# stella-cv/stella_vslam

Hardware: NVIDIA H100
Metric: frames/sec (ORB+match+local BA) @1920x1080, 2000 kpts (higher is better)
Workload: dtype u8

## Files before the change

### stella_vslam_b200/csrc/orb_kernels.cu

```cuda
#include <cuda.h>

#include <algorithm>
#include <cmath>
#include <new>
#include <vector>

#include "common.cuh"
#include "track_chain.cuh"
#include "util_trig.cuh"

namespace b200 {
namespace orb {

constexpr int kMaxLevels = 16;
constexpr int kBorder = 19;
constexpr int kCell = 64;
constexpr int kOverlap = 6;
constexpr int kTileMax = kCell + kOverlap;
constexpr int kTilePitch = 80;

struct LevelGeom {
    int w, h, pitch;
    unsigned long long offset;
    float sf;
    int nx, ny;
    double delta_x, delta_y;
    int grid_base;
    int ncols;
    float size;
    int tab_x, tab_y;
};

struct Geom {
    int num_levels;
    int grid_cells;
    int ini_thr, min_thr;
    LevelGeom lv[kMaxLevels];
};

struct CellDesc {
    unsigned short level, i, j, min_x, min_y, w, h, pad;
};

struct RawKp {
    short x, y;
    unsigned char m;
    unsigned char level;
    unsigned short pad;
};

struct ResizeTap {
    short ofs, w0, w1, pad;
};

struct Images {
    const unsigned char* img0;
    unsigned long long pitch0, fstride0;
    unsigned char* pyr;
    unsigned long long pyr_fstride;
};

__device__ __forceinline__ const unsigned char* level_ptr(const Images& im, const Geom& g, int level, int frame, int* pitch) {
    if (level == 0) {
        *pitch = (int)im.pitch0;
        return im.img0 + (size_t)frame * im.fstride0;
    }
    *pitch = g.lv[level].pitch;
    return im.pyr + (size_t)frame * im.pyr_fstride + g.lv[level].offset;
}

struct TmapSet {
    CUtensorMap m[kMaxLevels];
};

__device__ __forceinline__ unsigned smem_u32(const void* p) { return (unsigned)__cvta_generic_to_shared(p); }

__device__ __forceinline__ void mbar_init(unsigned long long* bar, unsigned count) {
    asm volatile("mbarrier.init.shared::cta.b64 [%0], %1;" ::"r"(smem_u32(bar)), "r"(count));
    asm volatile("fence.mbarrier_init.release.cluster;" ::: "memory");
}
__device__ __forceinline__ void mbar_expect_tx(unsigned long long* bar, unsigned bytes) {
    asm volatile("mbarrier.arrive.expect_tx.shared::cta.b64 _, [%0], %1;" ::"r"(smem_u32(bar)), "r"(bytes) : "memory");
}
__device__ __forceinline__ void mbar_wait(unsigned long long* bar, unsigned parity) {
    asm volatile(
        "{\n\t.reg .pred p;\n\t"
        "WAIT_%=:\n\t"
        "mbarrier.try_wait.parity.shared::cta.b64 p, [%0], %1;\n\t"
        "@p bra DONE_%=;\n\t"
        "bra WAIT_%=;\n\t"
        "DONE_%=:\n\t}" ::"r"(smem_u32(bar)),
        "r"(parity)
        : "memory");
}
__device__ __forceinline__ void tma_load_3d(void* smem_dst, const CUtensorMap* tmap, int x, int y, int z, unsigned long long* bar) {
    asm volatile("cp.async.bulk.tensor.3d.shared::cluster.global.mbarrier::complete_tx::bytes [%0], [%1, {%2, %3, %4}], [%5];" ::"r"(
                     smem_u32(smem_dst)),
                 "l"(reinterpret_cast<unsigned long long>(tmap)), "r"(x), "r"(y), "r"(z), "r"(smem_u32(bar))
                 : "memory");
}

constexpr int kRzRows = 8;

__global__ void __launch_bounds__(128) resize_kernel(const __grid_constant__ Geom g, Images im, const ResizeTap* __restrict__ taps, int level) {
    const LevelGeom& L = g.lv[level];
    const int frame = blockIdx.z;
    int spitch;
    const unsigned char* src = level_ptr(im, g, level - 1, frame, &spitch);
    unsigned char* dst = im.pyr + (size_t)frame * im.pyr_fstride + L.offset;
    const int sw = g.lv[level - 1].w, sh = g.lv[level - 1].h;
    const int dxq = (blockIdx.x * blockDim.x + threadIdx.x) * 4;
    const int dy0 = blockIdx.y * kRzRows;
    if (dxq >= L.pitch) return;
    const int n_valid = min(4, L.w - dxq);
    const unsigned store_mask = n_valid >= 4 ? 0xFFFFFFFFu : (n_valid <= 0 ? 0u : ((1u << (8 * n_valid)) - 1u));
    int ofs[4], ofs1[4];
    unsigned w01[4];
#pragma unroll
    for (int k = 0; k < 4; ++k) {
        const ResizeTap t = taps[L.tab_x + min(dxq + k, L.w - 1)];
        ofs[k] = t.ofs;
        ofs1[k] = min((int)t.ofs + 1, sw - 1);
        w01[k] = ((unsigned)t.w0 & 0xFFFFu) | ((unsigned)t.w1 << 16);
    }
    int rowA = -1, rowB = -1;
    unsigned hA[4] = {0, 0, 0, 0}, hB[4] = {0, 0, 0, 0};
    auto hrow = [&](int sy, unsigned (&h)[4]) {
        const unsigned char* r = src + (size_t)sy * spitch;
#pragma unroll
        for (int k = 0; k < 4; ++k) h[k] = __dp2a_lo(w01[k], (unsigned)r[ofs[k]] | ((unsigned)r[ofs1[k]] << 8), 0u) >> 4;
    };
    const int dy_end = min(dy0 + kRzRows, L.h);
    unsigned char* drow = dst + (size_t)dy0 * L.pitch + dxq;
    for (int dy = dy0; dy < dy_end; ++dy, drow += L.pitch) {
        const ResizeTap ty = taps[L.tab_y + dy];
        const int s0 = min(max((int)ty.ofs, 0), sh - 1), s1 = min(max((int)ty.ofs + 1, 0), sh - 1);
        if (s0 != rowA) {
            if (s0 == rowB) {
#pragma unroll
                for (int k = 0; k < 4; ++k) hA[k] = hB[k];
            } else {
                hrow(s0, hA);
            }
            rowA = s0;
        }
        if (s1 != rowB) {
            if (s1 == rowA) {
#pragma unroll
                for (int k = 0; k < 4; ++k) hB[k] = hA[k];
            } else {
                hrow(s1, hB);
            }
            rowB = s1;
        }
        const unsigned b0 = (unsigned)(int)ty.w0 << 16, b1 = (unsigned)(int)ty.w1 << 16;
        unsigned out = 0;
#pragma unroll
        for (int k = 0; k < 4; ++k) out |= ((__umulhi(b0, hA[k]) + __umulhi(b1, hB[k]) + 2u) >> 2) << (8 * k);
        *reinterpret_cast<unsigned*>(drow) = out & store_mask;
    }
}

__device__ __forceinline__ bool has_run9(unsigned m16) {
    unsigned m = m16 | (m16 << 16);
    unsigned x = m & (m >> 1);
    x &= x >> 2;
    x &= x >> 4;
    x &= m >> 8;
    return (x & 0xFFFFu) != 0;
}

#define FAST_OFF(k, P)                                                                                              \
    ((k) == 0 ? 3 * (P) : (k) == 1 ? 3 * (P) + 1 : (k) == 2 ? 2 * (P) + 2 : (k) == 3 ? (P) + 3 : (k) == 4 ? 3      \
     : (k) == 5 ? -(P) + 3 : (k) == 6 ? -2 * (P) + 2 : (k) == 7 ? -3 * (P) + 1 : (k) == 8 ? -3 * (P)              \
     : (k) == 9 ? -3 * (P)-1 : (k) == 10 ? -2 * (P)-2 : (k) == 11 ? -(P)-3 : (k) == 12 ? -3                        \
     : (k) == 13 ? (P)-3 : (k) == 14 ? 2 * (P)-2 : 3 * (P)-1)

__device__ __forceinline__ bool mask_zero(const unsigned char* mask, unsigned long long mask_pitch, unsigned y, unsigned x, float sf) {
    const int r = (int)__fmul_rn((float)y, sf), c = (int)__fmul_rn((float)x, sf);
    return mask[(size_t)r * mask_pitch + c] == 0;
}

__device__ __forceinline__ unsigned fast_m4(const unsigned (&w)[7][3], unsigned neg_tlow2) {
    constexpr int DX[16] = {0, 1, 2, 3, 3, 3, 2, 1, 0, -1, -2, -3, -3, -3, -2, -1};
    constexpr int DY[16] = {3, 3, 2, 1, 0, -1, -2, -3, -3, -3, -2, -1, 0, 1, 2, 3};
    unsigned pe[16], po[16];
    const unsigned ve = __byte_perm(w[3][1], 0, 0x4240), vo = __byte_perm(w[3][1], 0, 0x4341);
    auto extract = [&](int k) {
        const int dx = DX[k], r = DY[k] + 3;
        unsigned x;
        if (dx == 0) x = w[r][1];
        else if (dx > 0) x = __byte_perm(w[r][1], w[r][2], 0x3210 + 0x1111 * dx);
        else x = __byte_perm(w[r][0], w[r][1], 0x3210 + 0x1111 * (4 + dx));
        pe[k] = __byte_perm(x, 0, 0x4240);
        po[k] = __byte_perm(x, 0, 0x4341);
    };
#pragma unroll
    for (int k = 0; k < 16; ++k) extract(k);
    unsigned res[2];
#pragma unroll
    for (int half = 0; half < 2; ++half) {
        const unsigned* p = half ? po : pe;
        const unsigned v = half ? vo : ve;
        unsigned mx3[16], mn3[16];
#pragma unroll
        for (int k = 0; k < 16; ++k) {
            mx3[k] = __vimax3_u16x2(p[k], p[(k + 1) & 15], p[(k + 2) & 15]);
            mn3[k] = __vimin3_u16x2(p[k], p[(k + 1) & 15], p[(k + 2) & 15]);
        }
        unsigned mx9[16], mn9[16];
#pragma unroll
        for (int k = 0; k < 16; ++k) {
            mx9[k] = __vimax3_u16x2(mx3[k], mx3[(k + 3) & 15], mx3[(k + 6) & 15]);
            mn9[k] = __vimin3_u16x2(mn3[k], mn3[(k + 3) & 15], mn3[(k + 6) & 15]);
        }
        unsigned a = __vimin3_u16x2(mx9[0], mx9[1], mx9[2]), b = __vimax3_u16x2(mn9[0], mn9[1], mn9[2]);
#pragma unroll
        for (int k = 3; k < 15; k += 2) {
            a = __vimin3_u16x2(a, mx9[k], mx9[k + 1]);
            b = __vimax3_u16x2(b, mn9[k], mn9[k + 1]);
        }
        a = __vminu2(a, mx9[15]);
        b = __vmaxu2(b, mn9[15]);
        const unsigned dark = __vsub2(v, a), bright = __vsub2(b, v);
        const unsigned m = __vimax_s16x2_relu(dark, bright);
        res[half] = __viaddmax_s16x2_relu(m, neg_tlow2, 0u);
    }
    return __byte_perm(res[0], res[1], 0x6240);
}

__device__ __forceinline__ unsigned fast_candidates4(const unsigned (&w)[7][3], unsigned tlow2) {
    const unsigned x0 = w[6][1], x8 = w[0][1];
    const unsigned x4 = __byte_perm(w[3][1], w[3][2], 0x6543), x12 = __byte_perm(w[3][0], w[3][1], 0x4321);
    unsigned r[2];
#pragma unroll
    for (int half = 0; half < 2; ++half) {
        const unsigned sel = half ? 0x4341u : 0x4240u;
        const unsigned p0 = __byte_perm(x0, 0, sel), p8 = __byte_perm(x8, 0, sel), p4 = __byte_perm(x4, 0, sel), p12 = __byte_perm(x12, 0, sel);
        const unsigned v = __byte_perm(w[3][1], 0, sel);
        const unsigned hi = __vminu2(__vmaxu2(p0, p8), __vmaxu2(p4, p12));
        const unsigned lo = __vmaxu2(__vminu2(p0, p8), __vminu2(p4, p12));
        const unsigned vt = v + tlow2, lot = lo + tlow2;
        r[half] = (__vmaxu2(hi, vt) ^ vt) | (__vmaxu2(v, lot) ^ lot);
    }
    return ((r[0] & 0xFFFFu) ? 1u : 0u) | ((r[1] & 0xFFFFu) ? 2u : 0u) | ((r[0] >> 16) ? 4u : 0u) | ((r[1] >> 16) ? 8u : 0u);
}

__device__ __forceinline__ int fast_score1(const unsigned char* __restrict__ p, int t_low) {
    constexpr int OFF[16] = {3 * kTilePitch,     3 * kTilePitch + 1,  2 * kTilePitch + 2,  kTilePitch + 3,  3,  -kTilePitch + 3, -2 * kTilePitch + 2, -3 * kTilePitch + 1,
                             -3 * kTilePitch,    -3 * kTilePitch - 1, -2 * kTilePitch - 2, -kTilePitch - 3, -3, kTilePitch - 3,  2 * kTilePitch - 2,  3 * kTilePitch - 1};
    unsigned c[16];
#pragma unroll
    for (int k = 0; k < 16; ++k) c[k] = (unsigned)p[OFF[k]] * 0xFFFF0001u + 0x00FF0000u;
    const int v = p[0];
    unsigned mx3[16];
#pragma unroll
    for (int k = 0; k < 16; ++k) mx3[k] = __vimax3_s16x2(c[k], c[(k + 1) & 15], c[(k + 2) & 15]);
    unsigned ab = 0x00FF00FFu;
#pragma unroll
    for (int k = 0; k < 16; k += 2)
        ab = __vimin3_s16x2(ab, __vimax3_s16x2(mx3[k], mx3[(k + 3) & 15], mx3[(k + 6) & 15]),
                            __vimax3_s16x2(mx3[k + 1], mx3[(k + 4) & 15], mx3[(k + 7) & 15]));
    const int a = (int)(ab & 0xFFFFu), b = 255 - (int)(ab >> 16);
    const int at = a + t_low, vt = v + t_low;
    return (max(v, at) - at) + (max(b, vt) - vt);
}

constexpr int kFastThreads = 256;
constexpr int kTileRows = kTileMax + 2;
constexpr int kRawPitch = 96;

template <bool kUseTma>
__global__ void __launch_bounds__(kFastThreads) fast_cells_kernel(const __grid_constant__ Geom g, const __grid_constant__ TmapSet tmaps, Images im,
                                                                  const CellDesc* __restrict__ cells, const unsigned char* __restrict__ mask,
                                                                  unsigned long long mask_pitch, unsigned long long* __restrict__ grid,
                                                                  int arena_frame0, int* __restrict__ raw_corners) {
    __shared__ __align__(16) unsigned char tile[kTileRows * kTilePitch];
    __shared__ __align__(16) unsigned char mmap[kTileRows * kTilePitch];
    __shared__ __align__(128) unsigned char raw[kUseTma ? kTileRows * kRawPitch : 16];
    __shared__ __align__(8) unsigned long long tma_bar;
    __shared__ int skip;
    __shared__ unsigned short cand[(kTileMax - 6) * (kTileMax - 6)];
    __shared__ int n_cand;

    const CellDesc cd = cells[blockIdx.x];
    const int frame = blockIdx.y;
    const int level = cd.level;
    const LevelGeom& L = g.lv[level];
    const int cw = cd.w, ch = cd.h;
    const int tid = threadIdx.x;

    if (tid == 0) {
        int s = 0;
        if (mask) {
            const unsigned max_x = cd.min_x + cw, max_y = cd.min_y + ch;
            s = mask_zero(mask, mask_pitch, cd.min_y, cd.min_x, L.sf) || mask_zero(mask, mask_pitch, max_y, cd.min_x, L.sf)
                || mask_zero(mask, mask_pitch, cd.min_y, max_x, L.sf) || mask_zero(mask, mask_pitch, max_y, max_x, L.sf);
        }
        skip = s;
        n_cand = 0;
    }
    if constexpr (kUseTma) {
        if (tid == 0) {
            mbar_init(&tma_bar, 1);
            mbar_expect_tx(&tma_bar, kTileRows * kRawPitch);
            tma_load_3d(raw, &tmaps.m[level], (int)cd.min_x - 3, (int)cd.min_y, frame + (level ? arena_frame0 : 0), &tma_bar);
        }
        __syncthreads();
        mbar_wait(&tma_bar, 0);
        for (int idx = tid; idx < kTileRows * (kTilePitch / 4); idx += kFastThreads) {
            const int y = idx / (kTilePitch / 4), q = idx - y * (kTilePitch / 4);
            const unsigned* rw = reinterpret_cast<const unsigned*>(raw + y * kRawPitch) + q;
            reinterpret_cast<unsigned*>(tile)[idx] = __funnelshift_r(rw[0], rw[1], 16);
            reinterpret_cast<unsigned*>(mmap)[idx] = 0u;
        }
        __syncthreads();
    } else {
        int pitch;
        const unsigned char* src = level_ptr(im, g, level, frame, &pitch);
        src += (size_t)cd.min_y * pitch + cd.min_x;
        for (int idx = tid; idx < kTileRows * (kTilePitch / 4); idx += kFastThreads) {
            const int y = idx / (kTilePitch / 4), c4 = (idx - y * (kTilePitch / 4)) * 4;
            unsigned v = 0;
            if (y < ch) {
#pragma unroll
                for (int b = 0; b < 4; ++b) {
                    const int x = c4 + b - 1;
                    if (x >= 0 && x < cw) v |= (unsigned)src[(size_t)y * pitch + x] << (8 * b);
                }
            }
            reinterpret_cast<unsigned*>(tile)[idx] = v;
            reinterpret_cast<unsigned*>(mmap)[idx] = 0u;
        }
        __syncthreads();
    }
    if (skip) return;

    const int t_low = min(g.ini_thr, g.min_thr);
    const unsigned neg_tlow2 = (unsigned)((-t_low) & 0xFFFF) * 0x10001u;
    if (t_low <= 126) {
        const int wq = tid & 15, rg = tid >> 4;
        const int c0 = 4 + 4 * wq;
        const int lx0 = c0 - 1;
        const int y0 = 3 + 4 * rg;
        if (lx0 <= cw - 4 && y0 <= ch - 4) {
            const unsigned c7f = (unsigned)(0x7F - t_low) * 0x01010101u;
            auto gt = [&](unsigned d) { return (((d & 0x7F7F7F7Fu) + c7f) | d) & 0x80808080u; };
            unsigned ctr[10];
#pragma unroll
            for (int r = 0; r < 10; ++r) ctr[r] = *reinterpret_cast<const unsigned*>(tile + (y0 - 3 + r) * kTilePitch + c0);
            unsigned acc = 0;
#pragma unroll
            for (int i = 0; i < 4; ++i) {
                const unsigned* row = reinterpret_cast<const unsigned*>(tile + (y0 + i) * kTilePitch + c0 - 4);
                const unsigned v = ctr[i + 3];
                const unsigned p4 = __byte_perm(v, row[2], 0x6543), p12 = __byte_perm(row[0], v, 0x4321);
                const unsigned gbits = (gt(__vabsdiffu4(ctr[i + 6], v)) | gt(__vabsdiffu4(ctr[i], v))) & (gt(__vabsdiffu4(p4, v)) | gt(__vabsdiffu4(p12, v)));
                acc |= gbits >> (7 - i);
            }
            const int nvalid = min(4, cw - 3 - lx0), nrows = min(4, ch - 3 - y0);
            acc &= (0xFFFFFFFFu >> (32 - 8 * nvalid)) & (((1u << nrows) - 1u) * 0x01010101u);
            if (acc) {
                int pos = atomicAdd(&n_cand, __popc(acc));
                const unsigned enc0 = (unsigned)((y0 << 8) | c0);
#pragma unroll
                for (int b = 0; b < 4; ++b) {
                    const unsigned nib = (acc >> (8 * b)) & 0xFu;
#pragma unroll
                    for (int i = 0; i < 4; ++i)
                        if ((nib >> i) & 1u) cand[pos + __popc(nib & ((1u << i) - 1u))] = (unsigned short)(enc0 + (unsigned)((i << 8) | b));
                    pos += __popc(nib);
                }
            }
        }
    } else {
        const int wq = tid & 15, rg = tid >> 4;
        const int c0 = 4 + 4 * wq;
        const int lx0 = c0 - 1;
        const int y0 = 3 + 4 * rg;
        if (lx0 <= cw - 4 && y0 <= ch - 4) {
            unsigned w[10][3];
#pragma unroll
            for (int r = 0; r < 10; ++r) {
                const int y = y0 - 3 + r;
                const unsigned* row = reinterpret_cast<const unsigned*>(tile + y * kTilePitch + c0 - 4);
                w[r][0] = row[0];
                w[r][1] = row[1];
                w[r][2] = row[2];
            }
            const int nvalid = min(4, cw - 3 - lx0);
            const unsigned keep = (1u << nvalid) - 1u;
            unsigned bits = 0;
#pragma unroll
            for (int i = 0; i < 4; ++i) {
                if (y0 + i <= ch - 4) {
                    unsigned ww[7][3];
#pragma unroll
                    for (int r = 0; r < 7; ++r) {
                        ww[r][0] = w[i + r][0];
                        ww[r][1] = w[i + r][1];
                        ww[r][2] = w[i + r][2];
                    }
                    bits |= (fast_candidates4(ww, (unsigned)t_low * 0x10001u) & keep) << (4 * i);
                }
            }
            if (bits) {
                int pos = atomicAdd(&n_cand, __popc(bits));
                while (bits) {
                    const int k = __ffs(bits) - 1;
                    bits &= bits - 1;
                    cand[pos++] = (unsigned short)(((y0 + (k >> 2)) << 8) | (c0 + (k & 3)));
                }
            }
        }
    }
    __syncthreads();
    {
        const int n = n_cand;
        for (int i = tid; i < n; i += kFastThreads) {
            const int e = cand[i], y = e >> 8, c = e & 0xFF;
            mmap[y * kTilePitch + c] = (unsigned char)fast_score1(tile + y * kTilePitch + c, t_low);
        }
    }
    __syncthreads();
    const int ini_rel = g.ini_thr - t_low, min_rel = g.min_thr - t_low;
    const int n_c = n_cand;
// ... 264 lines not shown
            for (int idx = lane; idx < kFdHpW * 5; idx += 32) {
                const int rb = idx / kFdHpW, c = idx - rb * kFdHpW;
                unsigned p[7];
#pragma unroll
                for (int t = 0; t < 7; ++t) p[t] = (4 * rb + t < kFdHpRows) ? S.hp[(4 * rb + t) * kFdHpW + c] : 0u;
#pragma unroll
                for (int i = 0; i < 4; ++i) {
                    unsigned e = __dp2a_lo(p[i], E01, 0u);
                    e = __dp2a_hi(p[i + 1], E01, e);
                    e = __dp2a_lo(p[i + 2], E23, e);
                    e = __dp2a_hi(p[i + 3], E23, e);
                    unsigned o = __dp2a_lo(p[i], O01, 0u);
                    o = __dp2a_hi(p[i + 1], O01, o);
                    o = __dp2a_lo(p[i + 2], O23, o);
                    o = __dp2a_hi(p[i + 3], O23, o);
                    S.blur[(8 * rb + 2 * i) * kFdHpW + c] = (unsigned char)min((e + 32768u) >> 16, 255u);
                    S.blur[(8 * rb + 2 * i + 1) * kFdHpW + c] = (unsigned char)min((o + 32768u) >> 16, 255u);
                }
            }
        }
        int m10 = 0, m01 = 0;
        if (lane < 31) {
            const int u = lane - 15, au = abs(u);
            const unsigned char* c = tile + 21 * kFdTileW + ox + 21 + u;
            int col = 0;
#pragma unroll
            for (int v = -15; v <= 15; ++v) {
                if (au <= c_umax[v < 0 ? -v : v]) {
                    const int val = c[v * kFdTileW];
                    col += val;
                    m01 += v * val;
                }
            }
            m10 = u * col;
        }
#pragma unroll
        for (int s2 = 16; s2 > 0; s2 >>= 1) {
            m10 += __shfl_xor_sync(0xFFFFFFFFu, m10, s2);
            m01 += __shfl_xor_sync(0xFFFFFFFFu, m01, s2);
        }
        const float angle = fast_atan2_deg((float)m01, (float)m10);
        __syncwarp();
        const float arad = (float)((double)angle * 3.14159265358979323846 / 180.0);
        const float ca = util_cos(arad), sa = util_sin(arad);
        const unsigned char* bc = S.blur + kFdR * kFdHpW + kFdR;
        unsigned val = 0;
#pragma unroll
        for (int b = 0; b < 8; ++b) {
            const float x0 = (float)(int)(signed char)(pat[b] & 0xFF), y0 = (float)(int)(signed char)((pat[b] >> 8) & 0xFF);
            const float x1 = (float)(int)(signed char)((pat[b] >> 16) & 0xFF), y1 = (float)(int)(signed char)(pat[b] >> 24);
            int r0 = __float2int_rn(__fadd_rn(__fmul_rn(x0, sa), __fmul_rn(y0, ca)));
            int c0 = __float2int_rn(__fsub_rn(__fmul_rn(x0, ca), __fmul_rn(y0, sa)));
            int r1 = __float2int_rn(__fadd_rn(__fmul_rn(x1, sa), __fmul_rn(y1, ca)));
            int c1 = __float2int_rn(__fsub_rn(__fmul_rn(x1, ca), __fmul_rn(y1, sa)));
            r0 = max(-kFdR, min(kFdR, r0)); c0 = max(-kFdR, min(kFdR, c0));
            r1 = max(-kFdR, min(kFdR, r1)); c1 = max(-kFdR, min(kFdR, c1));
            val |= (unsigned)(bc[r0 * kFdHpW + c0] < bc[r1 * kFdHpW + c1]) << b;
        }
        const size_t o = (size_t)frame * out_stride + k;
        descs[o * 32 + lane] = (unsigned char)val;
        if (lane == 0) {
            b200_keypoint_t kp;
            float x = (float)kx, y = (float)ky;
            if (level > 0) {
                x = __fmul_rn(x, L.sf);
                y = __fmul_rn(y, L.sf);
            }
            kp.x = x;
            kp.y = y;
            kp.size = L.size;
            kp.angle = angle;
            kp.response = (float)(rk.m - 1);
            kp.octave = level;
            kps[o] = kp;
        }
        __syncwarp();
    }
}

static inline short sat_short_rint(float v) {
    long r = lrintf(v);
    return (short)std::min(32767L, std::max(-32768L, r));
}
static inline int floor_to_int(float v) {
    int i = (int)v;
    return i - (v < (float)i);
}

typedef CUresult (*EncodeTiledFn)(CUtensorMap*, CUtensorMapDataType, cuuint32_t, void*, const cuuint64_t*, const cuuint64_t*, const cuuint32_t*,
                                  const cuuint32_t*, CUtensorMapInterleave, CUtensorMapSwizzle, CUtensorMapL2promotion, CUtensorMapFloatOOBfill);

static EncodeTiledFn encode_tiled_fn() {
    static EncodeTiledFn fn = nullptr;
    static bool tried = false;
    if (!tried) {
        tried = true;
        void* p = nullptr;
        cudaDriverEntryPointQueryResult q;
        if (cudaGetDriverEntryPointByVersion("cuTensorMapEncodeTiled", &p, 12000, cudaEnableDefault, &q) == cudaSuccess
            && q == cudaDriverEntryPointSuccess)
            fn = (EncodeTiledFn)p;
    }
    return fn;
}

static bool make_level_tmap(CUtensorMap* out, const void* base, int w, int h, size_t pitch, size_t fstride, int frames, int box_w = kRawPitch,
                            int box_h = kTileRows) {
    EncodeTiledFn fn = encode_tiled_fn();
    if (!fn) return false;
    if ((reinterpret_cast<unsigned long long>(base) & 15ull) || (pitch & 15) || (frames > 1 && (fstride & 15)) || w < 1 || h < 1) return false;
    const cuuint64_t dims[3] = {(cuuint64_t)w, (cuuint64_t)h, (cuuint64_t)std::max(frames, 1)};
    const cuuint64_t strides[2] = {(cuuint64_t)pitch, (cuuint64_t)(frames > 1 ? fstride : pitch * (size_t)h + ((16 - (pitch * (size_t)h) % 16) % 16))};
    const cuuint32_t box[3] = {(cuuint32_t)box_w, (cuuint32_t)box_h, 1};
    const cuuint32_t estr[3] = {1, 1, 1};
    return fn(out, CU_TENSOR_MAP_DATA_TYPE_UINT8, 3, const_cast<void*>(base), dims, strides, box, estr, CU_TENSOR_MAP_INTERLEAVE_NONE,
              CU_TENSOR_MAP_SWIZZLE_NONE, CU_TENSOR_MAP_L2_PROMOTION_NONE, CU_TENSOR_MAP_FLOAT_OOB_FILL_NONE)
           == CUDA_SUCCESS;
}

struct Extractor {
    b200_orb_params_t prm{};
    std::vector<float> mask_rects;
    cudaStream_t own_stream = nullptr, stream = nullptr, copy_stream = nullptr;
    cudaEvent_t ev[8] = {};
    std::vector<cudaEvent_t> chunk_events;
    cudaEvent_t chunk_event(int i) {
        while ((int)chunk_events.size() <= i) {
            cudaEvent_t e = nullptr;
            if (cudaEventCreateWithFlags(&e, cudaEventDisableTiming) != cudaSuccess) return nullptr;
            chunk_events.push_back(e);
        }
        return chunk_events[i];
    }
    bool timing = false;
    float stage_ms[6] = {};
    int width = 0, height = 0, batch_cap = 0;
    Geom geom{};
    std::vector<float> sf;
    int n_cells = 0, raw_stride = 0;
    size_t pyr_fstride = 0, img0_pitch = 0, img0_fstride = 0;
    unsigned char *d_img0 = nullptr, *d_pyr = nullptr, *d_rect_mask = nullptr, *d_user_mask = nullptr;
    CellDesc* d_cells = nullptr;
    ResizeTap* d_taps = nullptr;
    unsigned long long* d_grid = nullptr;
    RawKp* d_raw = nullptr;
    int *d_counts = nullptr, *d_level_counts = nullptr, *d_raw_corners = nullptr;
    b200_keypoint_t* d_kps = nullptr;
    unsigned char* d_descs = nullptr;
    int* h_counts = nullptr;
    int last_batch = 0;
    const unsigned char* last_img0 = nullptr;
    size_t last_pitch0 = 0, last_fstride0 = 0;
    bool rect_mask_ready = false;
    TmapSet tmaps{};
    TmapSet tmaps_desc{};
    bool tmaps_ok = false, last_used_tma = false;
    int tmap_frames = 0;
    b200_keypoint_t* out_kps = nullptr;
    unsigned char* out_descs = nullptr;
    int* out_counts = nullptr;
    int out_stride = 0;
    b200_keypoint_t* res_kps() const { return out_kps ? out_kps : d_kps; }
    unsigned char* res_descs() const { return out_kps ? out_descs : d_descs; }
    int* res_counts() const { return out_kps ? out_counts : d_counts; }
    int res_stride() const { return out_kps ? out_stride : raw_stride; }

    void free_arenas() {
        cudaFree(d_img0); cudaFree(d_pyr); cudaFree(d_rect_mask); cudaFree(d_user_mask);
        cudaFree(d_cells); cudaFree(d_taps); cudaFree(d_grid); cudaFree(d_raw);
        cudaFree(d_counts); cudaFree(d_level_counts); cudaFree(d_raw_corners); cudaFree(d_kps); cudaFree(d_descs);
        if (h_counts) cudaFreeHost(h_counts);
        d_img0 = d_pyr = d_rect_mask = d_user_mask = nullptr;
        d_cells = nullptr; d_taps = nullptr; d_grid = nullptr; d_raw = nullptr;
        d_counts = d_level_counts = d_raw_corners = nullptr; d_kps = nullptr; d_descs = nullptr; h_counts = nullptr;
        rect_mask_ready = false;
    }

    static int level_geometry(const b200_orb_params_t& prm, int w, int h, Geom& g, std::vector<float>& sf) {
        const int nl = prm.num_levels;
        sf.assign(nl, 1.0f);
        for (int l = 1; l < nl; ++l) sf[l] = prm.scale_factor * sf[l - 1];
        g = Geom{};
        g.num_levels = nl;
        g.ini_thr = std::min(255, std::max(0, prm.ini_fast_thr));
        g.min_thr = std::min(255, std::max(0, prm.min_fast_thr));
        const unsigned min_area_sqrt = (unsigned)std::sqrt((double)prm.min_area);
        unsigned long long off = 0;
        int grid_base = 0;
        for (int l = 0; l < nl; ++l) {
            LevelGeom& L = g.lv[l];
            if (l == 0) {
                L.w = w;
                L.h = h;
            } else {
                const double scale = sf[l];
                L.w = (int)std::round(w * 1.0 / scale);
                L.h = (int)std::round(h * 1.0 / scale);
            }
            if (L.w < 1 || L.h < 1) {
                set_error("pyramid level %d of a %dx%d image is empty", l, w, h);
                return B200_ERR_INVALID;
            }
            L.pitch = round_up(L.w, 64);
            L.offset = off;
            off += round_up((unsigned long long)L.pitch * L.h, 256ull);
            L.sf = sf[l];
            L.size = (float)(unsigned)(31 * sf[l]);
            L.grid_base = grid_base;
            if (L.w > 2 * kBorder && L.h > 2 * kBorder) {
                const int span_x = L.w - 2 * kBorder, span_y = L.h - 2 * kBorder;
                const double s = (double)((float)min_area_sqrt / sf[l]);
                L.nx = (int)(unsigned)std::ceil(span_x / s);
                L.ny = (int)(unsigned)std::ceil(span_y / s);
                L.delta_x = (double)span_x / L.nx;
                L.delta_y = (double)span_y / L.ny;
                L.ncols = span_x / kCell + 1;
            } else {
                L.nx = L.ny = 0;
                L.delta_x = L.delta_y = 1.0;
                L.ncols = 1;
            }
            grid_base += L.nx * L.ny;
        }
        g.grid_cells = grid_base;
        return B200_OK;
    }

    int configure(int w, int h, int batch) {
        if (w == width && h == height && batch <= batch_cap) return B200_OK;
        B200_CUDA(cudaStreamSynchronize(stream));
        free_arenas();
        width = height = batch_cap = 0;
        int rc = level_geometry(prm, w, h, geom, sf);
        if (rc) return rc;
        const int nl = geom.num_levels;
        std::vector<CellDesc> cells;
        std::vector<ResizeTap> taps;
        for (int l = 0; l < nl; ++l) {
            LevelGeom& L = geom.lv[l];
            if (L.w > 2 * kBorder && L.h > 2 * kBorder) {
                const unsigned max_bx = L.w - kBorder, max_by = L.h - kBorder;
                const unsigned ncols = (max_bx - kBorder) / kCell + 1, nrows = (max_by - kBorder) / kCell + 1;
                for (unsigned i = 0; i < nrows; ++i) {
                    const unsigned min_y = kBorder + i * kCell;
                    if (max_by - kOverlap <= min_y) continue;
                    const unsigned max_y = std::min(min_y + kCell + kOverlap, max_by);
                    for (unsigned j = 0; j < ncols; ++j) {
                        const unsigned min_x = kBorder + j * kCell;
                        if (max_bx - kOverlap <= min_x) continue;
                        const unsigned max_x = std::min(min_x + kCell + kOverlap, max_bx);
                        CellDesc c{};
                        c.level = (unsigned short)l; c.i = (unsigned short)i; c.j = (unsigned short)j;
                        c.min_x = (unsigned short)min_x; c.min_y = (unsigned short)min_y;
                        c.w = (unsigned short)(max_x - min_x); c.h = (unsigned short)(max_y - min_y);
                        cells.push_back(c);
                    }
                }
            }
            if (l > 0) {
                const LevelGeom& S = geom.lv[l - 1];
                const double inv_sx = (double)L.w / S.w, inv_sy = (double)L.h / S.h;
                const double scale_x = 1. / inv_sx, scale_y = 1. / inv_sy;
                L.tab_x = (int)taps.size();
                for (int dx = 0; dx < L.w; ++dx) {
                    float fx = (float)((dx + 0.5) * scale_x - 0.5);
                    int sx = floor_to_int(fx);
                    fx -= sx;
                    if (sx < 0) { fx = 0; sx = 0; }
                    if (sx >= S.w - 1) { fx = 0; sx = S.w - 1; }
                    taps.push_back(ResizeTap{(short)sx, sat_short_rint((1.f - fx) * 2048.f), sat_short_rint(fx * 2048.f), 0});
                }
                L.tab_y = (int)taps.size();
                for (int dy = 0; dy < L.h; ++dy) {
                    float fy = (float)((dy + 0.5) * scale_y - 0.5);
                    int sy = floor_to_int(fy);
                    fy -= sy;
                    taps.push_back(ResizeTap{(short)sy, sat_short_rint((1.f - fy) * 2048.f), sat_short_rint(fy * 2048.f), 0});
                }
            }
        }
        if (geom.lv[0].w > 32767 || geom.lv[0].h > 32767) {
            set_error("image %dx%d too large", w, h);
            return B200_ERR_INVALID;
        }
        n_cells = (int)cells.size();
        raw_stride = std::max(1, geom.grid_cells);
        unsigned long long total = 0;
        for (int l = 0; l < nl; ++l) total = geom.lv[l].offset + round_up((unsigned long long)geom.lv[l].pitch * geom.lv[l].h, 256ull);
        pyr_fstride = total;
        img0_pitch = geom.lv[0].pitch;
        img0_fstride = (size_t)img0_pitch * h;

        B200_CUDA(cudaMalloc(&d_img0, img0_fstride * batch));
        B200_CUDA(cudaMalloc(&d_pyr, pyr_fstride * batch));
        B200_CUDA(cudaMalloc(&d_user_mask, img0_fstride));
        B200_CUDA(cudaMalloc(&d_cells, sizeof(CellDesc) * std::max(1, n_cells)));
        B200_CUDA(cudaMalloc(&d_taps, sizeof(ResizeTap) * std::max<size_t>(1, taps.size())));
        B200_CUDA(cudaMalloc(&d_grid, sizeof(unsigned long long) * (size_t)raw_stride * batch));
        B200_CUDA(cudaMalloc(&d_raw, sizeof(RawKp) * (size_t)raw_stride * batch));
        B200_CUDA(cudaMalloc(&d_counts, sizeof(int) * batch));
        B200_CUDA(cudaMalloc(&d_level_counts, sizeof(int) * kMaxLevels * batch));
        B200_CUDA(cudaMalloc(&d_raw_corners, sizeof(int) * batch));
        B200_CUDA(cudaMalloc(&d_kps, sizeof(b200_keypoint_t) * (size_t)raw_stride * batch));
        B200_CUDA(cudaMalloc(&d_descs, (size_t)32 * raw_stride * batch));
        B200_CUDA(cudaHostAlloc(&h_counts, sizeof(int) * (kMaxLevels + 1) * batch, cudaHostAllocDefault));
        if (n_cells) B200_CUDA(cudaMemcpyAsync(d_cells, cells.data(), sizeof(CellDesc) * n_cells, cudaMemcpyHostToDevice, stream));
        if (!taps.empty()) B200_CUDA(cudaMemcpyAsync(d_taps, taps.data(), sizeof(ResizeTap) * taps.size(), cudaMemcpyHostToDevice, stream));
        if (!mask_rects.empty()) {
            std::vector<unsigned char> m((size_t)img0_pitch * h, 255);
            for (size_t r = 0; r + 3 < mask_rects.size(); r += 4) {
                const unsigned x_min = (unsigned)std::round(w * mask_rects[r]), x_max = (unsigned)std::round(w * mask_rects[r + 1]);
                const unsigned y_min = (unsigned)std::round(h * mask_rects[r + 2]), y_max = (unsigned)std::round(h * mask_rects[r + 3]);
                for (unsigned y = y_min; y <= y_max && y < (unsigned)h; ++y)
                    for (unsigned x = x_min; x <= x_max && x < (unsigned)w; ++x) m[(size_t)y * img0_pitch + x] = 0;
            }
            B200_CUDA(cudaMalloc(&d_rect_mask, (size_t)img0_pitch * h));
            B200_CUDA(cudaMemcpyAsync(d_rect_mask, m.data(), m.size(), cudaMemcpyHostToDevice, stream));
            B200_CUDA(cudaStreamSynchronize(stream));
            rect_mask_ready = true;
        }
        B200_CUDA(cudaStreamSynchronize(stream));
        tmaps_ok = true;
        tmap_frames = batch;
        for (int l = 1; l < nl && tmaps_ok; ++l)
            tmaps_ok = make_level_tmap(&tmaps.m[l], d_pyr + geom.lv[l].offset, geom.lv[l].w, geom.lv[l].h, geom.lv[l].pitch, pyr_fstride, batch)
                       && make_level_tmap(&tmaps_desc.m[l], d_pyr + geom.lv[l].offset, geom.lv[l].w, geom.lv[l].h, geom.lv[l].pitch, pyr_fstride, batch,
                                          kFdTileW, kFdIn);
        width = w;
        height = h;
        batch_cap = batch;
        return B200_OK;
    }

    int run(const void* d_images, size_t pitch, size_t fstride, int batch, const void* d_mask, size_t mask_pitch, int frame0 = 0,
            bool record = true) {
        Images im{(const unsigned char*)d_images, pitch, fstride, d_pyr + (size_t)frame0 * pyr_fstride, pyr_fstride};
        last_img0 = (const unsigned char*)d_images - (size_t)frame0 * fstride;
        last_pitch0 = pitch;
        last_fstride0 = fstride;
        const unsigned char* mask = (const unsigned char*)d_mask;
        unsigned long long mpitch = mask_pitch;
        if (!mask && rect_mask_ready) {
            mask = d_rect_mask;
            mpitch = img0_pitch;
        }
        if (out_kps && out_stride < geom.grid_cells) {
            set_error("bound output stride %d is smaller than the keypoint upper bound %d", out_stride, geom.grid_cells);
            return B200_ERR_CAPACITY;
        }
        const int nl = geom.num_levels;
        const bool tm = timing && record;
        unsigned long long* grid = d_grid + (size_t)frame0 * geom.grid_cells;
        RawKp* raw = d_raw + (size_t)frame0 * raw_stride;
        int* counts = res_counts() + frame0;
        if (tm) B200_CUDA(cudaEventRecord(ev[0], stream));
        for (int l = 1; l < nl; ++l) {
            const LevelGeom& L = geom.lv[l];
            dim3 grd(ceil_div(L.pitch / 4, 128), ceil_div(L.h, kRzRows), batch);
            resize_kernel<<<grd, 128, 0, stream>>>(geom, im, d_taps, l);
        }
        if (tm) B200_CUDA(cudaEventRecord(ev[1], stream));
        B200_CUDA(cudaMemsetAsync(grid, 0, sizeof(unsigned long long) * (size_t)std::max(1, geom.grid_cells) * batch, stream));
        B200_CUDA(cudaMemsetAsync(d_raw_corners + frame0, 0, sizeof(int) * batch, stream));
        if (n_cells) {
            const bool tma = tmaps_ok && make_level_tmap(&tmaps.m[0], d_images, geom.lv[0].w, geom.lv[0].h, pitch, fstride, batch);
            if (tma) fast_cells_kernel<true><<<dim3(n_cells, batch), kFastThreads, 0, stream>>>(geom, tmaps, im, d_cells, mask, mpitch, grid, frame0,
                                                                                                   d_raw_corners + frame0);
            else fast_cells_kernel<false><<<dim3(n_cells, batch), kFastThreads, 0, stream>>>(geom, tmaps, im, d_cells, mask, mpitch, grid, frame0,
                                                                                                    d_raw_corners + frame0);
            last_used_tma = tma;
        }
        if (tm) B200_CUDA(cudaEventRecord(ev[2], stream));
        select_kernel<<<dim3(nl, batch), 256, 0, stream>>>(geom, grid, raw, raw_stride, counts, d_level_counts + (size_t)frame0 * kMaxLevels);
        if (tm) B200_CUDA(cudaEventRecord(ev[3], stream));
        if (tm) B200_CUDA(cudaEventRecord(ev[4], stream));
        {
            const size_t smem = sizeof(FdWarp) * kDescWarps;
            const bool tma = tmaps_ok
                             && make_level_tmap(&tmaps_desc.m[0], d_images, geom.lv[0].w, geom.lv[0].h, pitch, fstride, batch, kFdTileW, kFdIn);
            b200_keypoint_t* okps = res_kps() + (size_t)frame0 * res_stride();
            unsigned char* odesc = res_descs() + (size_t)frame0 * res_stride() * 32;
            if (tma) {
                B200_CUDA(cudaFuncSetAttribute(describe_kernel<true>, cudaFuncAttributeMaxDynamicSharedMemorySize, (int)smem));
                describe_kernel<true><<<dim3(kDescBlocksPerFrame, batch), kDescWarps * 32, smem, stream>>>(geom, tmaps_desc, im, raw, raw_stride, counts, okps,
                                                                                                          odesc, res_stride(), frame0);
            } else {
                B200_CUDA(cudaFuncSetAttribute(describe_kernel<false>, cudaFuncAttributeMaxDynamicSharedMemorySize, (int)smem));
                describe_kernel<false><<<dim3(kDescBlocksPerFrame, batch), kDescWarps * 32, smem, stream>>>(geom, tmaps_desc, im, raw, raw_stride, counts, okps,
                                                                                                           odesc, res_stride(), frame0);
            }
        }
        if (tm) B200_CUDA(cudaEventRecord(ev[5], stream));
        B200_CUDA(cudaGetLastError());
        last_batch = frame0 + batch;
        return B200_OK;
    }
};

struct CamModel {
    int model;
    double fx, fy, cx, cy, k1, k2, p1, p2, k3, cols, rows;
};
__device__ __forceinline__ void undistort_point(const CamModel& c, const b200_keypoint_t& kp, float& ux, float& uy) {
    ux = kp.x;
    uy = kp.y;
    if (c.model == 0) {
        const double ifx = 1. / c.fx, ify = 1. / c.fy;
        const double u = kp.x, v = kp.y;
        double x = (u - c.cx) * ifx, y = (v - c.cy) * ify;
        const double x0 = x, y0 = y;
        double error = 1.7976931348623157e308;
        for (int j = 0; j < 20 && !(error < 1e-6); ++j) {
            double r2 = x * x + y * y;
            const double icdist = 1.0 / (1 + ((c.k3 * r2 + c.k2) * r2 + c.k1) * r2);
            if (icdist < 0) {
                x = (u - c.cx) * ifx;
                y = (v - c.cy) * ify;
                break;
            }
            const double deltaX = 2 * c.p1 * x * y + c.p2 * (r2 + 2 * x * x);
            const double deltaY = c.p1 * (r2 + 2 * y * y) + 2 * c.p2 * x * y;
            x = (x0 - deltaX) * icdist;
            y = (y0 - deltaY) * icdist;
            r2 = x * x + y * y;
            const double r4 = r2 * r2, r6 = r4 * r2;
            const double a1 = 2 * x * y, a2 = r2 + 2 * x * x, a3 = r2 + 2 * y * y;
            const double cdist = 1 + c.k1 * r2 + c.k2 * r4 + c.k3 * r6;
            const double xd0 = x * cdist + c.p1 * a1 + c.p2 * a2, yd0 = y * cdist + c.p1 * a3 + c.p2 * a1;
            const double ex = (xd0 * c.fx + c.cx) - u, ey = (yd0 * c.fy + c.cy) - v;
            error = sqrt(ex * ex + ey * ey);
        }
        ux = (float)(c.fx * x + c.cx);
        uy = (float)(c.fy * y + c.cy);
    }
}

__global__ void __launch_bounds__(128) undistort_bearings_kernel(CamModel c, const b200_keypoint_t* __restrict__ in, int n,
                                                                 b200_keypoint_t* __restrict__ out, double* __restrict__ bearings) {
    const int i = blockIdx.x * blockDim.x + threadIdx.x;
    if (i >= n) return;
    const b200_keypoint_t kp = in[i];
    float ux, uy;
    undistort_point(c, kp, ux, uy);
    if (out) {
        b200_keypoint_t o;
        o.x = ux;
        o.y = uy;
        o.size = kp.size;
        o.angle = kp.angle;
        o.response = (c.model == 0) ? 0.f : kp.response;
        o.octave = kp.octave;
        out[i] = o;
    }
    if (bearings) {
        double* b = bearings + 3 * (size_t)i;
        if (c.model == 1) {
            const double kTwoPi = 2.0 * 3.14159265358979323846, kPi = 3.14159265358979323846;
            const double lon = ((double)__fdiv_rn(ux, (float)(unsigned)c.cols) - 0.5) * kTwoPi;
            const double lat = -((double)__fdiv_rn(uy, (float)(unsigned)c.rows) - 0.5) * kPi;
            b[0] = cos(lat) * sin(lon);
            b[1] = -sin(lat);
            b[2] = cos(lat) * cos(lon);
        } else {
            const double xn = ((double)ux - c.cx) / c.fx, yn = ((double)uy - c.cy) / c.fy;
            const double l2 = sqrt(xn * xn + yn * yn + 1.0);
            b[0] = xn / l2;
            b[1] = yn / l2;
            b[2] = 1.0 / l2;
        }
    }
}

template <int kChannels>
__global__ void __launch_bounds__(256) gray_kernel(const unsigned char* __restrict__ src, unsigned long long spitch, unsigned long long sframe,
                                                   unsigned char* __restrict__ dst, unsigned long long dpitch, unsigned long long dframe, int w, int h,
                                                   int rgb_order) {
    const int gx = blockIdx.x * blockDim.x + threadIdx.x, y = blockIdx.y, f = blockIdx.z;
    const int x0 = gx * 4;
    if (x0 >= w) return;
    const unsigned char* srow = src + (size_t)f * sframe + (size_t)y * spitch;
    unsigned char* drow = dst + (size_t)f * dframe + (size_t)y * dpitch;
    const unsigned cr = rgb_order ? 9798u : 3735u, cb = rgb_order ? 3735u : 9798u;
    if (x0 + 4 <= w) {
        const unsigned* p = reinterpret_cast<const unsigned*>(srow + (size_t)x0 * kChannels);
        unsigned px[4];
        if (kChannels == 4) {
            px[0] = p[0]; px[1] = p[1]; px[2] = p[2]; px[3] = p[3];
        } else {
            const unsigned a = p[0], b = p[1], c = p[2];
            px[0] = a;
            px[1] = __funnelshift_r(a, b, 24);
            px[2] = __funnelshift_r(b, c, 16);
            px[3] = c >> 8;
        }
        unsigned out = 0;
#pragma unroll
        for (int k = 0; k < 4; ++k) {
            const unsigned c0 = px[k] & 0xFF, c1 = (px[k] >> 8) & 0xFF, c2 = (px[k] >> 16) & 0xFF;
            out |= ((c0 * cr + c1 * 19235u + c2 * cb + (1u << 14)) >> 15) << (8 * k);
        }
        *reinterpret_cast<unsigned*>(drow + x0) = out;
    } else {
        for (int x = x0; x < w; ++x) {
            const unsigned char* q = srow + (size_t)x * kChannels;
            drow[x] = (unsigned char)((q[0] * cr + q[1] * 19235u + q[2] * cb + (1u << 14)) >> 15);
        }
    }
}

template <int kChannels>
__global__ void __launch_bounds__(128) gray16_kernel(const unsigned char* __restrict__ src, unsigned long long spitch, unsigned long long sframe,
                                                     unsigned char* __restrict__ dst, unsigned long long dpitch, unsigned long long dframe, int w, int h,
// ... 722 lines not shown
```

Baseline: 9441.

## Stage resize source rows in shared memory and plan rows per level

The pyramid resize kernel now cooperatively loads the needed source rows of each output tile into shared memory, using 16-byte vector loads when aligned, and samples from shared memory instead of doing scattered byte loads from global memory. A host-side planner picks the number of output rows per block and the smem pitch per level so the staging fits in shared memory. The FAST kernel also gains a min-blocks-per-SM launch bound of 8, which may force register limits. This adds a block-wide sync and staging overhead, and the pyramid resize is a small part of the full pipeline.

```diff
diff --git a/stella_vslam_b200/csrc/orb_kernels.cu b/stella_vslam_b200/csrc/orb_kernels.cu
--- a/stella_vslam_b200/csrc/orb_kernels.cu
+++ b/stella_vslam_b200/csrc/orb_kernels.cu
@@ -100,17 +100,45 @@
                  : "memory");
 }
 
-constexpr int kRzRows = 8;
-
-__global__ void __launch_bounds__(128) resize_kernel(const __grid_constant__ Geom g, Images im, const ResizeTap* __restrict__ taps, int level) {
+constexpr int kRzThreads = 128;
+constexpr int kRzCols = 4 * kRzThreads;
+constexpr int kRzRowsMax = 16;
+
+__global__ void __launch_bounds__(kRzThreads) resize_kernel(const __grid_constant__ Geom g, Images im, const ResizeTap* __restrict__ taps, int level,
+                                                            int rows, int sp) {
+    extern __shared__ __align__(16) unsigned char srows[];
     const LevelGeom& L = g.lv[level];
     const int frame = blockIdx.z;
     int spitch;
     const unsigned char* src = level_ptr(im, g, level - 1, frame, &spitch);
     unsigned char* dst = im.pyr + (size_t)frame * im.pyr_fstride + L.offset;
     const int sw = g.lv[level - 1].w, sh = g.lv[level - 1].h;
-    const int dxq = (blockIdx.x * blockDim.x + threadIdx.x) * 4;
-    const int dy0 = blockIdx.y * kRzRows;
+    const int dx_tile = blockIdx.x * kRzCols;
+    const int dxq = dx_tile + threadIdx.x * 4;
+    const int dy0 = blockIdx.y * rows;
+    const int dy_end = min(dy0 + rows, L.h);
+    const int sx_lo = taps[L.tab_x + min(dx_tile, L.w - 1)].ofs;
+    const int sx_hi = min((int)taps[L.tab_x + min(dx_tile + kRzCols - 1, L.w - 1)].ofs + 1, sw - 1);
+    const int sy_lo = min(max((int)taps[L.tab_y + dy0].ofs, 0), sh - 1);
+    const int sy_hi = min(max((int)taps[L.tab_y + dy_end - 1].ofs + 1, 0), sh - 1);
+    const bool vec = ((reinterpret_cast<unsigned long long>(src) | (unsigned long long)spitch) & 15ull) == 0;
+    const int sbase = vec ? (sx_lo & ~15) : sx_lo;
+    const int nrows = sy_hi - sy_lo + 1;
+    const unsigned char* s0row = src + (size_t)sy_lo * spitch + sbase;
+    if (vec) {
+        const int nw = ((sx_hi - sbase) >> 4) + 1;
+        for (int i = threadIdx.x; i < nrows * nw; i += kRzThreads) {
+            const int r = i / nw, c = i - r * nw;
+            *reinterpret_cast<uint4*>(srows + r * sp + 16 * c) = __ldg(reinterpret_cast<const uint4*>(s0row + (size_t)r * spitch) + c);
+        }
+    } else {
+        const int nb = sx_hi - sbase + 1;
+        for (int i = threadIdx.x; i < nrows * nb; i += kRzThreads) {
+            const int r = i / nb, c = i - r * nb;
+            srows[r * sp + c] = __ldg(s0row + (size_t)r * spitch + c);
+        }
+    }
+    __syncthreads();
     if (dxq >= L.pitch) return;
     const int n_valid = min(4, L.w - dxq);
     const unsigned store_mask = n_valid >= 4 ? 0xFFFFFFFFu : (n_valid <= 0 ? 0u : ((1u << (8 * n_valid)) - 1u));
@@ -119,18 +147,17 @@
 #pragma unroll
     for (int k = 0; k < 4; ++k) {
         const ResizeTap t = taps[L.tab_x + min(dxq + k, L.w - 1)];
-        ofs[k] = t.ofs;
-        ofs1[k] = min((int)t.ofs + 1, sw - 1);
+        ofs[k] = t.ofs - sbase;
+        ofs1[k] = min((int)t.ofs + 1, sw - 1) - sbase;
         w01[k] = ((unsigned)t.w0 & 0xFFFFu) | ((unsigned)t.w1 << 16);
     }
     int rowA = -1, rowB = -1;
     unsigned hA[4] = {0, 0, 0, 0}, hB[4] = {0, 0, 0, 0};
     auto hrow = [&](int sy, unsigned (&h)[4]) {
-        const unsigned char* r = src + (size_t)sy * spitch;
+        const unsigned char* r = srows + (sy - sy_lo) * sp;
 #pragma unroll
         for (int k = 0; k < 4; ++k) h[k] = __dp2a_lo(w01[k], (unsigned)r[ofs[k]] | ((unsigned)r[ofs1[k]] << 8), 0u) >> 4;
     };
-    const int dy_end = min(dy0 + kRzRows, L.h);
     unsigned char* drow = dst + (size_t)dy0 * L.pitch + dxq;
     for (int dy = dy0; dy < dy_end; ++dy, drow += L.pitch) {
         const ResizeTap ty = taps[L.tab_y + dy];
@@ -271,7 +298,7 @@
 constexpr int kRawPitch = 96;
 
 template <bool kUseTma>
-__global__ void __launch_bounds__(kFastThreads) fast_cells_kernel(const __grid_constant__ Geom g, const __grid_constant__ TmapSet tmaps, Images im,
+__global__ void __launch_bounds__(kFastThreads, 8) fast_cells_kernel(const __grid_constant__ Geom g, const __grid_constant__ TmapSet tmaps, Images im,
                                                                   const CellDesc* __restrict__ cells, const unsigned char* __restrict__ mask,
                                                                   unsigned long long mask_pitch, unsigned long long* __restrict__ grid,
                                                                   int arena_frame0, int* __restrict__ raw_corners) {
@@ -842,6 +869,8 @@
     const unsigned char* last_img0 = nullptr;
     size_t last_pitch0 = 0, last_fstride0 = 0;
     bool rect_mask_ready = false;
+    int rz_rows[kMaxLevels] = {}, rz_sp[kMaxLevels] = {};
+    size_t rz_smem[kMaxLevels] = {};
     TmapSet tmaps{};
     TmapSet tmaps_desc{};
     bool tmaps_ok = false, last_used_tma = false;
@@ -914,6 +943,30 @@
         }
         g.grid_cells = grid_base;
         return B200_OK;
+    }
+
+    void resize_plan(const std::vector<ResizeTap>& taps, int l) {
+        const LevelGeom &L = geom.lv[l], &S = geom.lv[l - 1];
+        int span = 1;
+        for (int x0 = 0; x0 < L.pitch; x0 += kRzCols) {
+            const int lo = taps[L.tab_x + std::min(x0, L.w - 1)].ofs;
+            const int hi = std::min(taps[L.tab_x + std::min(x0 + kRzCols - 1, L.w - 1)].ofs + 1, S.w - 1);
+            span = std::max(span, hi - lo + 1);
+        }
+        const int sp = round_up(span + 15, 16);
+        auto clip = [&](int y) { return std::min(std::max(y, 0), S.h - 1); };
+        for (int rows = kRzRowsMax;; rows /= 2) {
+            int nrows = 1;
+            for (int y0 = 0; y0 < L.h; y0 += rows)
+                nrows = std::max(nrows, clip(taps[L.tab_y + std::min(y0 + rows, L.h) - 1].ofs + 1) - clip(taps[L.tab_y + y0].ofs) + 1);
+            const size_t smem = (size_t)nrows * sp;
+            if (smem <= 48 * 1024 || rows == 1) {
+                rz_rows[l] = rows;
+                rz_sp[l] = sp;
+                rz_smem[l] = smem;
+                return;
+            }
+        }
     }
 
     int configure(int w, int h, int batch) {
@@ -973,6 +1026,12 @@
             set_error("image %dx%d too large", w, h);
             return B200_ERR_INVALID;
         }
+        size_t rz_smem_max = 0;
+        for (int l = 1; l < nl; ++l) {
+            resize_plan(taps, l);
+            rz_smem_max = std::max(rz_smem_max, rz_smem[l]);
+        }
+        if (rz_smem_max > 48 * 1024) B200_CUDA(cudaFuncSetAttribute(resize_kernel, cudaFuncAttributeMaxDynamicSharedMemorySize, (int)rz_smem_max));
         n_cells = (int)cells.size();
         raw_stride = std::max(1, geom.grid_cells);
         unsigned long long total = 0;
@@ -1046,8 +1105,8 @@
         if (tm) B200_CUDA(cudaEventRecord(ev[0], stream));
         for (int l = 1; l < nl; ++l) {
             const LevelGeom& L = geom.lv[l];
-            dim3 grd(ceil_div(L.pitch / 4, 128), ceil_div(L.h, kRzRows), batch);
-            resize_kernel<<<grd, 128, 0, stream>>>(geom, im, d_taps, l);
+            dim3 grd(ceil_div(L.pitch, kRzCols), ceil_div(L.h, rz_rows[l]), batch);
+            resize_kernel<<<grd, kRzThreads, rz_smem[l], stream>>>(geom, im, d_taps, l, rz_rows[l], rz_sp[l]);
         }
         if (tm) B200_CUDA(cudaEventRecord(ev[1], stream));
         B200_CUDA(cudaMemsetAsync(grid, 0, sizeof(unsigned long long) * (size_t)std::max(1, geom.grid_cells) * batch, stream));
```

After: 9566 (median of 6 runs). No clear change (+1.3%).
